# adhney/video-quierer

Hardware: AMD Instinct MI355X
Metric: frames/sec CLIP ViT-B/32 encode + queries/sec top-10 over 1M×512 embeds (higher is better)
Workload: dtype fp16 MFMA operands (every GEMM group), fp32 accumulate

## Files before the change

### video-quierer_amd/csrc/encoder_kernels.h

```cpp
#pragma once
#include "vq_common.h"
#include "gemm_mfma.h"

namespace vq {


template <bool F16>
__device__ __forceinline__ uint2 pack4_h(f32x4 v) {
    if constexpr (F16) {
        typedef __attribute__((ext_vector_type(4))) _Float16 h4;
        h4 b = {(_Float16)v[0], (_Float16)v[1], (_Float16)v[2], (_Float16)v[3]};
        return __builtin_bit_cast(uint2, b);
    } else {
        typedef __attribute__((ext_vector_type(4))) __bf16 bf16x4;
        bf16x4 b = {(__bf16)v[0], (__bf16)v[1], (__bf16)v[2], (__bf16)v[3]};
        return __builtin_bit_cast(uint2, b);
    }
}
template <bool F16>
__host__ __device__ inline uint16_t to_h16(float f) {
    if constexpr (F16) return __builtin_bit_cast(uint16_t, (_Float16)f);
    else return f32_to_bf16_rne(f);
}

// ... 342 lines not shown
#pragma unroll
    for (int i = 0; i < NV; ++i) {
        v[i].x -= mean; v[i].y -= mean; v[i].z -= mean; v[i].w -= mean;
        q += (v[i].x * v[i].x + v[i].y * v[i].y) + (v[i].z * v[i].z + v[i].w * v[i].w);
    }
    const float rstd = rsqrtf(wave_sum(q) / (float)hidden + eps);
#pragma unroll
    for (int i = 0; i < NV; ++i) {
        const float4 gg = *(const float4*)(g + (i * 64 + lane) * 4);
        const float4 bb = *(const float4*)(b + (i * 64 + lane) * 4);
        v[i].x = v[i].x * rstd * gg.x + bb.x; v[i].y = v[i].y * rstd * gg.y + bb.y;
        v[i].z = v[i].z * rstd * gg.z + bb.z; v[i].w = v[i].w * rstd * gg.w + bb.w;
    }
}

template <int NV, bool F16>
__global__ __launch_bounds__(256)
void layernorm_bf16_kernel(const float* __restrict__ x, uint16_t* __restrict__ h,
                           const float* __restrict__ g, const float* __restrict__ b,
                           int rows, float eps, int in_row_stride = 1) {
    constexpr int H = NV * 256;
    const int lane = threadIdx.x & 63;
    const int row = blockIdx.x * 4 + (threadIdx.x >> 6);
    if (row >= rows) return;
    float4 v[NV];
#pragma unroll
    for (int i = 0; i < NV; ++i) v[i] = *(const float4*)(x + (size_t)row * in_row_stride * H + (i * 64 + lane) * 4);
    ln_row<NV>(v, g, b, lane, eps, H);
#pragma unroll
    for (int i = 0; i < NV; ++i)
        *(uint2*)(h + (size_t)row * H + (i * 64 + lane) * 4) = pack4_h<F16>(f32x4{v[i].x, v[i].y, v[i].z, v[i].w});
}

template <int NV, bool F16>
__device__ __forceinline__ void emit_xh_and_partials(const float4 (&v)[NV], uint16_t* __restrict__ xh_row, LnPartials part,
                                                     int row, int lane) {
#pragma unroll
    for (int i = 0; i < NV; ++i) {
        *(uint2*)(xh_row + (i * 64 + lane) * 4) = pack4_h<F16>(f32x4{v[i].x, v[i].y, v[i].z, v[i].w});
        float s1 = (v[i].x + v[i].y) + (v[i].z + v[i].w);
        float s2 = (v[i].x * v[i].x + v[i].y * v[i].y) + (v[i].z * v[i].z + v[i].w * v[i].w);
        s1 = row16_sum(s1); s2 = row16_sum(s2);
        if ((lane & 15) == 0) part.ps[(size_t)(i * 4 + (lane >> 4)) * part.stride + row] = float2{s1, s2};
    }
}

template <int NV, bool F16>
__global__ __launch_bounds__(256)
void embed_finish_kernel(float* __restrict__ x, uint16_t* __restrict__ xh,
                         const float* __restrict__ cls, const float* __restrict__ pos0,
                         const float* __restrict__ g_pre, const float* __restrict__ b_pre,
                         LnPartials part, int rows, int tokens, float eps) {
    constexpr int H = NV * 256;
    const int lane = threadIdx.x & 63;
    const int row = blockIdx.x * 4 + (threadIdx.x >> 6);
    if (row >= rows) return;
    const bool is_cls = (row % tokens) == 0;
    float4 v[NV];
#pragma unroll
    for (int i = 0; i < NV; ++i) {
        const int o = (i * 64 + lane) * 4;
        if (is_cls) {
            const float4 c = *(const float4*)(cls + o), p = *(const float4*)(pos0 + o);
            v[i] = float4{c.x + p.x, c.y + p.y, c.z + p.z, c.w + p.w};
        } else {
            v[i] = *(const float4*)(x + (size_t)row * H + o);
        }
    }
    ln_row<NV>(v, g_pre, b_pre, lane, eps, H);
#pragma unroll
    for (int i = 0; i < NV; ++i) *(float4*)(x + (size_t)row * H + (i * 64 + lane) * 4) = v[i];
    emit_xh_and_partials<NV, F16>(v, xh + (size_t)row * H, part, row, lane);
}

inline __global__ __launch_bounds__(256)
void gather_rows_h16_kernel(const uint16_t* __restrict__ src, uint16_t* __restrict__ dst, int rows, int cols, int stride) {
    const int per_row = cols / 8;
    for (int i = blockIdx.x * blockDim.x + threadIdx.x; i < rows * per_row; i += gridDim.x * blockDim.x) {
        const int r = i / per_row, c = i - r * per_row;
        *(uint4*)(dst + (size_t)r * cols + c * 8) = *(const uint4*)(src + (size_t)r * stride * cols + c * 8);
    }
}

template <int NV, bool F16>
__global__ __launch_bounds__(256)
void embed_tokens_kernel(const int* __restrict__ ids, const float* __restrict__ tok, const float* __restrict__ pos,
                         float* __restrict__ x, uint16_t* __restrict__ xh, LnPartials part,
                         int rows, int seq, int vocab) {
    constexpr int H = NV * 256;
    const int lane = threadIdx.x & 63;
    const int row = blockIdx.x * 4 + (threadIdx.x >> 6);
    if (row >= rows) return;
    int id = ids[row];
    id = id < 0 ? 0 : (id >= vocab ? vocab - 1 : id);
    const int t = row % seq;
    float4 v[NV];
#pragma unroll
    for (int i = 0; i < NV; ++i) {
        const int o = (i * 64 + lane) * 4;
        const float4 a = *(const float4*)(tok + (size_t)id * H + o), p = *(const float4*)(pos + (size_t)t * H + o);
        v[i] = float4{a.x + p.x, a.y + p.y, a.z + p.z, a.w + p.w};
        *(float4*)(x + (size_t)row * H + o) = v[i];
    }
    emit_xh_and_partials<NV, F16>(v, xh + (size_t)row * H, part, row, lane);
}

inline __global__ void eos_rows_kernel(const int* __restrict__ ids, int* __restrict__ row_index, int n, int seq, int eos_id) {
    const int s = blockIdx.x * blockDim.x + threadIdx.x;
    if (s >= n) return;
    const int* p = ids + (size_t)s * seq;
    int pos = 0;
    if (eos_id == 2) {
        int best = p[0];
        for (int t = 1; t < seq; ++t) if (p[t] > best) { best = p[t]; pos = t; }
    } else {
        for (int t = 0; t < seq; ++t) if (p[t] == eos_id) { pos = t; break; }
    }
    row_index[s] = s * seq + pos;
}

#ifndef VQ_ATT_NT_LOAD
#define VQ_ATT_NT_LOAD 0
#endif
__device__ __forceinline__ uint4 ld16_att(const uint16_t* p) {
#if VQ_ATT_NT_LOAD
    typedef __attribute__((ext_vector_type(4))) unsigned int u32x4;
    const u32x4 v = __builtin_nontemporal_load((const u32x4*)p);
    return uint4{v[0], v[1], v[2], v[3]};
#else
    return *(const uint4*)p;
#endif
}

template <bool F16>
__global__ __launch_bounds__(256)
void attention_t64_kernel(const uint16_t* __restrict__ qkv, uint16_t* __restrict__ out,
                          int tokens, int hidden, int heads) {
    __shared__ __attribute__((aligned(16))) uint16_t vlds[4][64 * 64];
    const int lane = threadIdx.x & 63;
    const int wave = __builtin_amdgcn_readfirstlane(threadIdx.x >> 6);
    const int hgroups = heads >> 2;
    const int img = blockIdx.x / hgroups;
    const int head = (blockIdx.x - img * hgroups) * 4 + wave;
    const int ld = 3 * hidden;
    const uint16_t* base = qkv + (size_t)img * tokens * ld + head * 64;
    const int r16 = lane & 15, g = lane >> 4;
    typedef mfma_op<F16> op;
    typedef typename op::frag frag;

    uint16_t* vt = vlds[wave];
#pragma unroll
    for (int it = 0; it < 8; ++it) {
        const int id = it * 64 + lane, row = id >> 3, c = id & 7;
        uint4 val = {0u, 0u, 0u, 0u};
        if (row < tokens) val = ld16_att(base + 2 * hidden + (size_t)row * ld + c * 8);
        *(uint4*)(vt + row * 64 + c * 8) = val;
    }

    frag kf[4][2], qf[4][2];
#pragma unroll
    for (int t = 0; t < 4; ++t) {
        const int row = t * 16 + r16;
#pragma unroll
        for (int ks = 0; ks < 2; ++ks) {
            uint4 kv = {0u, 0u, 0u, 0u}, qv = {0u, 0u, 0u, 0u};
            if (row < tokens) {
// ... 18 lines not shown

    float inv_sum[4];
#pragma unroll
    for (int nt = 0; nt < 4; ++nt) {
        float mx = -3.0e38f;
#pragma unroll
        for (int mt = 0; mt < 4; ++mt)
#pragma unroll
            for (int r = 0; r < 4; ++r) {
                const int key = mt * 16 + g * 4 + r;
                if (key >= tokens) s[mt][nt][r] = -3.0e38f;
                mx = fmaxf(mx, s[mt][nt][r]);
            }
        mx = rows4_max(mx);
        float sum = 0.f;
#pragma unroll
        for (int mt = 0; mt < 4; ++mt)
#pragma unroll
            for (int r = 0; r < 4; ++r) {
                const float p = __expf(s[mt][nt][r] - mx);
                s[mt][nt][r] = p;
                sum += p;
            }
        sum = rows4_sum(sum);
        inv_sum[nt] = 1.0f / sum;
    }

    frag pf[4][2];
#pragma unroll
    for (int nt = 0; nt < 4; ++nt)
#pragma unroll
        for (int ss = 0; ss < 2; ++ss) {
            const f32x4 lo = s[2 * ss][nt], hi = s[2 * ss + 1][nt];
            const uint2 plo = pack4_h<F16>(lo), phi = pack4_h<F16>(hi);
            pf[nt][ss] = __builtin_bit_cast(frag, uint4{plo.x, plo.y, phi.x, phi.y});
        }

    __syncthreads();

    const int q4 = r16 >> 2, p4 = r16 & 3;
    typedef __attribute__((address_space(3))) s16x4 lds_s16x4;
#pragma unroll
    for (int dt = 0; dt < 4; ++dt) {
        f32x4 o[4];
#pragma unroll
        for (int nt = 0; nt < 4; ++nt) o[nt] = f32x4{0.f, 0.f, 0.f, 0.f};
#pragma unroll
        for (int ss = 0; ss < 2; ++ss) {
            const int key0 = 32 * ss + 4 * g + q4;
            const s16x4 lo = __builtin_amdgcn_ds_read_tr16_b64_v4i16(
                (lds_s16x4*)(vt + (key0) * 64 + dt * 16 + p4 * 4));
            const s16x4 hi = __builtin_amdgcn_ds_read_tr16_b64_v4i16(
                (lds_s16x4*)(vt + (key0 + 16) * 64 + dt * 16 + p4 * 4));
            typedef __attribute__((ext_vector_type(8))) short s16x8;
            const s16x8 both = {lo[0], lo[1], lo[2], lo[3], hi[0], hi[1], hi[2], hi[3]};
            const frag vf = __builtin_bit_cast(frag, both);
#pragma unroll
            for (int nt = 0; nt < 4; ++nt)
                o[nt] = op::run(vf, pf[nt][ss], o[nt]);
        }
#pragma unroll
        for (int nt = 0; nt < 4; ++nt) {
            const int qrow = nt * 16 + r16;
            if (qrow < tokens) {
                f32x4 v = o[nt];
                v[0] *= inv_sum[nt]; v[1] *= inv_sum[nt]; v[2] *= inv_sum[nt]; v[3] *= inv_sum[nt];
                *(uint2*)(out + ((size_t)img * tokens + qrow) * hidden + head * 64 + dt * 16 + g * 4) =
                    pack4_h<F16>(v);
            }
        }
    }
}

template <bool F16>
__device__ __forceinline__ typename mfma_op<F16>::frag ones_frag() {
    if constexpr (F16) { const _Float16 o = (_Float16)1.0f; return f16x8{o, o, o, o, o, o, o, o}; }
    else { const __bf16 o = (__bf16)1.0f; return bf16x8{o, o, o, o, o, o, o, o}; }
}
__device__ __forceinline__ uint4 buf_ld16(__amdgpu_buffer_rsrc_t r, int voff, int imm) {
    typedef __attribute__((ext_vector_type(4))) unsigned int u32x4;
    const u32x4 v = __builtin_amdgcn_raw_buffer_load_b128(r, voff + imm, 0, 0);
    return uint4{v[0], v[1], v[2], v[3]};
}
template <bool F16, int T>
__global__ __launch_bounds__(256, 2)
void attention_tile_kernel(const uint16_t* __restrict__ qkv, uint16_t* __restrict__ out, int hidden, int heads) {
    static_assert(T >= 17 && T <= 64, "single key tile of 64");
    __shared__ __attribute__((aligned(1024))) uint16_t vlds[4][64 * 64];
    typedef mfma_op<F16> op;
    typedef typename op::frag frag;
    typedef __attribute__((address_space(3))) void lds_void;
    const int lane = threadIdx.x & 63;
    const int wave = __builtin_amdgcn_readfirstlane(threadIdx.x >> 6);
    const int hgroups = heads >> 2;
    const int img = blockIdx.x / hgroups;
    const int head = (blockIdx.x - img * hgroups) * 4 + wave;
    const int ld = 3 * hidden;
    const int r16 = lane & 15, g = lane >> 4;
    const __amdgpu_buffer_rsrc_t src = __builtin_amdgcn_make_buffer_rsrc(
        (void*)(qkv + (size_t)img * T * ld + head * 64), 0, ((T - 1) * ld + 2 * hidden + 64) * 2, 0x00020000);
    const __amdgpu_buffer_rsrc_t dst = __builtin_amdgcn_make_buffer_rsrc(
        (void*)(out + (size_t)img * T * hidden + head * 64), 0, ((T - 1) * hidden + 64) * 2, 0x00020000);
    uint16_t* vt = vlds[wave];

    const int row_bytes = ld * 2;
    const int kq_off = r16 * row_bytes + g * 16;
    uint4 kraw[4][2], qraw[4][2];
#pragma unroll
    for (int t = 0; t < 4; ++t) {
        const int o = kq_off + t * 16 * row_bytes;
#pragma unroll
        for (int ks = 0; ks < 2; ++ks) {
            kraw[t][ks] = buf_ld16(src, o + hidden * 2, ks * 64);
            qraw[t][ks] = buf_ld16(src, o, ks * 64);
        }
    }
    constexpr int PIECES = (T + 7) / 8, ZROW0 = (T / 8) * 8;
    __builtin_amdgcn_sched_barrier(0);
    if constexpr (ZROW0 < 64) {
#pragma unroll
        for (int i = 0; i < (64 - ZROW0) * 128 / 1024; ++i)
            *(uint4*)(vt + ZROW0 * 64 + i * 512 + lane * 8) = uint4{0u, 0u, 0u, 0u};
    }
    const int v_off = (lane >> 3) * row_bytes + hidden * 4 + (((lane & 7) ^ (((lane >> 4) & 3) << 1)) << 4);
#pragma unroll
    for (int it = 0; it < PIECES; ++it) {
        if (it * 8 >= ZROW0) asm volatile("s_waitcnt lgkmcnt(0)" ::: "memory");
        __builtin_amdgcn_raw_ptr_buffer_load_lds(src, (lds_void*)(vt + it * 512), 16, v_off + it * 8 * row_bytes, 0, 0, 0);
    }
    __builtin_amdgcn_sched_barrier(0);

    frag kf[4][2], qf[4][2];
#pragma unroll
    for (int t = 0; t < 4; ++t)
#pragma unroll
        for (int ks = 0; ks < 2; ++ks) {
            kf[t][ks] = __builtin_bit_cast(frag, kraw[t][ks]);
            qf[t][ks] = __builtin_bit_cast(frag, qraw[t][ks]);
        }
    constexpr int KT = (T + 15) / 16;
    constexpr int FT = T / 16, R = T % 16;
    f32x4 s[4][4];
#pragma unroll
    for (int mt = 0; mt < KT; ++mt)
#pragma unroll
        for (int nt = 0; nt < 4; ++nt) {
            f32x4 a = {0.f, 0.f, 0.f, 0.f};
            a = op::run(kf[mt][0], qf[nt][0], a);
            a = op::run(kf[mt][1], qf[nt][1], a);
            s[mt][nt] = a;
        }
    const float NEGBIG = -3.0e38f, L2E = 1.44269504088896341f;
    float inv_sum[4];
#pragma unroll
    for (int nt = 0; nt < 4; ++nt) {
        float mx = NEGBIG;
#pragma unroll
        for (int mt = 0; mt < KT; ++mt)
#pragma unroll
            for (int r = 0; r < 4; ++r) {
                if (mt == FT) {
                    if (r >= R) continue;
                    if (4 * g + r >= R) s[mt][nt][r] = NEGBIG;
                }
                mx = fmaxf(mx, s[mt][nt][r]);
            }
        mx = rows4_max(mx);
        const float m2 = mx * L2E;
#pragma unroll
        for (int mt = 0; mt < KT; ++mt) {
            f32x4 e = s[mt][nt] * L2E - m2;
#pragma unroll
            for (int r = 0; r < 4; ++r) e[r] = (mt == FT && r >= R) ? 0.f : __builtin_amdgcn_exp2f(e[r]);
            s[mt][nt] = e;
        }
    }
    frag pf[4][2];
#pragma unroll
    for (int nt = 0; nt < 4; ++nt)
#pragma unroll
        for (int ss = 0; ss < 2; ++ss) {
            const uint2 plo = 2 * ss < KT ? pack4_h<F16>(s[2 * ss][nt]) : uint2{0u, 0u};
            const uint2 phi = 2 * ss + 1 < KT ? pack4_h<F16>(s[2 * ss + 1][nt]) : uint2{0u, 0u};
            pf[nt][ss] = __builtin_bit_cast(frag, uint4{plo.x, plo.y, phi.x, phi.y});
        }
    {
        const frag ones = ones_frag<F16>();
#pragma unroll
        for (int nt = 0; nt < 4; ++nt) {
            f32x4 d = {0.f, 0.f, 0.f, 0.f};
#pragma unroll
            for (int ss = 0; ss < 2; ++ss)
                if (2 * ss < KT) d = op::run(ones, pf[nt][ss], d);
            inv_sum[nt] = __builtin_amdgcn_rcpf(d[0]);
        }
    }

    __builtin_amdgcn_sched_barrier(0);
    asm volatile("s_waitcnt vmcnt(0)" ::: "memory");

    const int q4 = r16 >> 2, p4 = r16 & 3;
    const int sw = (2 * (g & 1) + (q4 >> 1)) & 3;
    typedef __attribute__((address_space(3))) s16x4 lds_s16x4;
    typedef __attribute__((ext_vector_type(8))) short s16x8;
    typedef __attribute__((ext_vector_type(4))) unsigned int u32x4;
    const int o_off = (r16 * hidden + g * 8) * 2;
#pragma unroll
    for (int a = 0; a < 2; ++a) {
        f32x4 o[2][4];
#pragma unroll
        for (int b = 0; b < 2; ++b) {
            const uint16_t* vrow = vt + (4 * g + q4) * 64 + (((4 * a + p4) ^ (sw << 1)) << 3) + 4 * b;
#pragma unroll
            for (int nt = 0; nt < 4; ++nt) o[b][nt] = f32x4{0.f, 0.f, 0.f, 0.f};
#pragma unroll
            for (int ss = 0; ss < 2; ++ss) {
                if (2 * ss >= KT) continue;
                const s16x4 lo = __builtin_amdgcn_ds_read_tr16_b64_v4i16((lds_s16x4*)(vrow + (32 * ss) * 64));
                s16x4 hi = {0, 0, 0, 0};
                if (2 * ss + 1 < KT) hi = __builtin_amdgcn_ds_read_tr16_b64_v4i16((lds_s16x4*)(vrow + (32 * ss + 16) * 64));
                const s16x8 both = {lo[0], lo[1], lo[2], lo[3], hi[0], hi[1], hi[2], hi[3]};
                const frag vf = __builtin_bit_cast(frag, both);
#pragma unroll
                for (int nt = 0; nt < 4; ++nt) o[b][nt] = op::run(vf, pf[nt][ss], o[b][nt]);
            }
        }
#pragma unroll
        for (int nt = 0; nt < 4; ++nt) {
            if (nt * 16 >= T) continue;
            const uint2 lo = pack4_h<F16>(o[0][nt] * inv_sum[nt]), hi = pack4_h<F16>(o[1][nt] * inv_sum[nt]);
            __builtin_amdgcn_raw_buffer_store_b128(u32x4{lo.x, lo.y, hi.x, hi.y}, dst, o_off + nt * 16 * hidden * 2 + a * 64, 0, 0);
        }
    }
}

template <bool F16, bool CAUSAL>
__global__ __launch_bounds__(256)
void attention_stream_kernel(const uint16_t* __restrict__ qkv, uint16_t* __restrict__ out,
                             int tokens, int hidden, int heads, int q_tiles, int total_units) {
    __shared__ __attribute__((aligned(16))) uint16_t vlds[4][64 * 64];
    typedef mfma_op<F16> op;
    typedef typename op::frag frag;
    const int lane = threadIdx.x & 63;
    const int wave = __builtin_amdgcn_readfirstlane(threadIdx.x >> 6);
    const int unit = blockIdx.x * 4 + wave;
    if (unit >= total_units) return;
    const int qt = unit % q_tiles;
    const int ih = unit / q_tiles;
    const int head = ih % heads, img = ih / heads;
    const int ld = 3 * hidden;
    const uint16_t* base = qkv + (size_t)img * tokens * ld + head * 64;
    const int r16 = lane & 15, g = lane >> 4;
    const int q0 = qt * 64;
    uint16_t* vt = vlds[wave];

    frag qf[4][2];
#pragma unroll
    for (int t = 0; t < 4; ++t) {
        const int row = q0 + t * 16 + r16;
#pragma unroll
        for (int ks = 0; ks < 2; ++ks) {
            uint4 qv = {0u, 0u, 0u, 0u};
            if (row < tokens) qv = *(const uint4*)(base + (size_t)row * ld + ks * 32 + g * 8);
            qf[t][ks] = __builtin_bit_cast(frag, qv);
        }
    }
    f32x4 o[4][4];
#pragma unroll
    for (int i = 0; i < 4; ++i)
#pragma unroll
        for (int j = 0; j < 4; ++j) o[i][j] = f32x4{0.f, 0.f, 0.f, 0.f};
    const float NEGBIG = -3.0e38f;
    float m_run[4] = {NEGBIG, NEGBIG, NEGBIG, NEGBIG}, l_run[4] = {0.f, 0.f, 0.f, 0.f};

    const int k_tiles = CAUSAL ? qt + 1 : (tokens + 63) / 64;
    const int q4 = r16 >> 2, p4 = r16 & 3;
    typedef __attribute__((address_space(3))) s16x4 lds_s16x4;
    typedef __attribute__((ext_vector_type(8))) short s16x8;

    for (int kt = 0; kt < k_tiles; ++kt) {
        const int k0 = kt * 64;
#pragma unroll
        for (int it = 0; it < 8; ++it) {
            const int id = it * 64 + lane, row = id >> 3, c = id & 7;
            uint4 val = {0u, 0u, 0u, 0u};
            if (k0 + row < tokens) val = *(const uint4*)(base + 2 * hidden + (size_t)(k0 + row) * ld + c * 8);
            *(uint4*)(vt + row * 64 + c * 8) = val;
        }
        frag kf[4][2];
#pragma unroll
        for (int t = 0; t < 4; ++t) {
            const int row = k0 + t * 16 + r16;
#pragma unroll
            for (int ks = 0; ks < 2; ++ks) {
                uint4 kv = {0u, 0u, 0u, 0u};
                if (row < tokens) kv = *(const uint4*)(base + hidden + (size_t)row * ld + ks * 32 + g * 8);
                kf[t][ks] = __builtin_bit_cast(frag, kv);
            }
        }
        f32x4 sc[4][4];
#pragma unroll
        for (int mt = 0; mt < 4; ++mt)
#pragma unroll
            for (int nt = 0; nt < 4; ++nt) {
                f32x4 a = {0.f, 0.f, 0.f, 0.f};
                a = op::run(kf[mt][0], qf[nt][0], a);
                a = op::run(kf[mt][1], qf[nt][1], a);
                sc[mt][nt] = a;
            }
        float alpha[4];
#pragma unroll
        for (int nt = 0; nt < 4; ++nt) {
            const int query = q0 + nt * 16 + r16;
            float mx = NEGBIG;
// ... 355 lines not shown
```

### video-quierer_amd/csrc/vq_encoder.hip

```cpp
#include "../../include/vq_amd.h"
#include "vq_common.h"
#include "gemm_dispatch.h"
#include "encoder_kernels.h"

#include <cmath>
#include <cstring>
#include <cstdlib>
#include <memory>
#include <mutex>
#include <type_traits>
#include <thread>
#include <algorithm>
#include <vector>

namespace vq {
int require_init();

enum EncClass { C_PATCHIFY = 0, C_GEMM_PATCH, C_EMBED_FINISH, C_LAYERNORM, C_GEMM_QKV, C_ATTENTION,
                C_GEMM_OUT, C_GEMM_FC1, C_GEMM_FC2, C_POOL, C_LAST_CLS };
static const char* kEncClassNames[VQ_ENC_NCLASS] = {
    "patchify_u8", "gemm_patch_embed", "embed_finish_ln", "layernorm_bf16", "gemm_qkv",
    "attention", "gemm_out_proj_residual", "gemm_fc1_quickgelu", "gemm_fc2_residual", "pool_project",
    "last_block_cls_rows"};

struct LayerW {
    float *c1_qkv, *c2_qkv, *b_out, *c1_fc1, *c2_fc1, *b_fc2;
    uint16_t *w_qkv, *w_out, *w_fc1, *w_fc2;
};

struct Arena {
    char* base = nullptr; size_t size = 0, used = 0;
    template <class T> T* take(size_t count) {
        used = (used + 255) & ~(size_t)255;
        T* p = (T*)(base + used);
        used += count * sizeof(T);
        return p;
    }
};

}

using namespace vq;

struct vq_encoder {
    vq_vit_config cfg{};
    int tokens = 0, patches = 0, grid = 0, patch_k = 0, max_batch = 0;
    int64_t rows_pad = 0, prow_pad = 0;
    hipStream_t stream = nullptr;
    hipStream_t own_stream = nullptr;
    std::mutex mu;
    Arena arena;
    std::shared_ptr<void> arena_owner;
    std::shared_ptr<void> weights_owner;
    uint16_t* w_patch = nullptr; float *b_patch = nullptr, *cls = nullptr, *pos = nullptr;
    float *pre_g = nullptr, *pre_b = nullptr, *post_g = nullptr, *post_b = nullptr, *w_proj = nullptr;
    std::vector<LayerW> layers;
    uint8_t* d_frames = nullptr;
    float *x = nullptr, *d_out = nullptr;
    uint16_t *h = nullptr, *qkv = nullptr, *att = nullptr, *mlp = nullptr;
    uint16_t* xl = nullptr;
    bool split_resid = true;
    float2* ps = nullptr;
    uint8_t* h_stage[2] = {nullptr, nullptr};
    float* h_out_stage = nullptr;
    uint8_t* d_slot_frames[2] = {nullptr, nullptr};
    float* h_slot_out[2] = {nullptr, nullptr};
    hipStream_t copy_stream = nullptr;
    hipEvent_t ev_h2d[2] = {nullptr, nullptr}, ev_fwd[2] = {nullptr, nullptr}, ev_done[2] = {nullptr, nullptr};
    int slot_n[2] = {0, 0};
    int run_layers = -1;
    bool keep_stream = false;
    bool stream_split = false;
    int last_n = 0;
    bool is_text = false;
    float* tok_emb = nullptr; int* d_ids = nullptr; int* d_rowidx = nullptr; int vocab = 0, eos_id = 0;
    bool attn_simple = false;
    bool attn_q64 = false;
    bool attn_t64 = false;
    bool prune_last = true;
    float patch_unscale = 1.0f;
    int f16_mask = 0;
    bool h_is_f16 = false;
    int gemm24_mask = 0;
    int gemm_force = GK_AUTO;
    bool profiling = false;
    struct Ev { int cls; hipEvent_t a, b; };
    std::vector<Ev> events;
    std::vector<hipEvent_t> pool;
};

namespace {

struct Prof {
    vq_encoder* e; int cls; hipEvent_t a = nullptr, b = nullptr;
    static hipEvent_t get(vq_encoder* e) {
        if (!e->pool.empty()) { hipEvent_t ev = e->pool.back(); e->pool.pop_back(); return ev; }
        hipEvent_t ev; (void)hipEventCreate(&ev); return ev;
    }
    Prof(vq_encoder* enc, int c) : e(enc), cls(c) {
        if (e->profiling) { a = get(e); b = get(e); (void)hipEventRecord(a, e->stream); }
    }
    ~Prof() {
        if (e->profiling) { (void)hipEventRecord(b, e->stream); e->events.push_back({cls, a, b}); }
    }
};

size_t arena_bytes(const vq_vit_config& c, int tokens, int patches, int patch_k, int max_batch,
                   int64_t rows_pad, int64_t prow_pad) {
    size_t h = c.hidden, m = c.mlp, n = 0;
    auto add = [&](size_t bytes) { n = ((n + 255) & ~(size_t)255) + bytes; };
    add((size_t)h * patch_k * 2); add(h * 4); add(h * 4); add((size_t)tokens * h * 4);
    add(h * 4); add(h * 4); add(h * 4); add(h * 4); add((size_t)c.proj_dim * h * 4);
    for (int l = 0; l < c.layers; ++l) {
        add(3 * h * 4); add(3 * h * 4); add(h * 4); add(m * 4); add(m * 4); add(h * 4);
        add(3 * h * h * 2); add(h * h * 2); add(m * h * 2); add(h * m * 2);
    }
    add((size_t)max_batch * c.image_size * c.image_size * 3);
    add((size_t)LN_MAX_GRANULES * rows_pad * 8);
    add((size_t)rows_pad * h * 4); add((size_t)max_batch * c.proj_dim * 4);
    add((size_t)rows_pad * h * 2); add((size_t)rows_pad * h * 2); add((size_t)rows_pad * 3 * h * 2); add((size_t)rows_pad * h * 2);
    size_t mlp_elems = std::max((size_t)rows_pad * m, (size_t)prow_pad * patch_k);
    add(mlp_elems * 2);
    (void)patches;
    return n + 4096;
}

int upload_f32(float* dst, const float* src, size_t n) {
    VQ_HIP(hipMemcpy(dst, src, n * 4, hipMemcpyHostToDevice));
    return 0;
}
int upload_h16(uint16_t* dst, const float* src, size_t n, bool f16, float scale = 1.0f) {
    std::vector<uint16_t> tmp(n);
    if (f16) for (size_t i = 0; i < n; ++i) tmp[i] = __builtin_bit_cast(uint16_t, (_Float16)(src[i] * scale));
    else     for (size_t i = 0; i < n; ++i) tmp[i] = f32_to_bf16_rne(src[i] * scale);
    VQ_HIP(hipMemcpy(dst, tmp.data(), n * 2, hipMemcpyHostToDevice));
    return 0;
}

enum : int { DT_PATCH = 1, DT_QKV = 2, DT_ATTN = 4, DT_FC1 = 8, DT_FC2 = 16, DT_ALL = 31 };

int upload_folded(uint16_t* dst, float* c1_dst, float* c2_dst, const float* W, const float* gamma, const float* beta,
                  const float* bias, size_t N, size_t K, bool f16, float scale = 1.0f) {
    std::vector<uint16_t> w16(N * K);
    std::vector<float> c1(N), c2(N);
    for (size_t n = 0; n < N; ++n) {
        double s1 = 0.0, s2 = 0.0;
        for (size_t k = 0; k < K; ++k) {
            const float wf = W[n * K + k] * scale * gamma[k];
            const uint16_t r = f16 ? __builtin_bit_cast(uint16_t, (_Float16)wf) : f32_to_bf16_rne(wf);
            w16[n * K + k] = r;
            s1 += f16 ? (double)(float)__builtin_bit_cast(_Float16, r) : (double)bf16_to_f32(r);
            s2 += (double)beta[k] * (double)W[n * K + k];
        }
        c1[n] = (float)s1;
        c2[n] = (float)((s2 + (double)bias[n]) * (double)scale);
    }
    VQ_HIP(hipMemcpy(dst, w16.data(), w16.size() * 2, hipMemcpyHostToDevice));
    VQ_HIP(hipMemcpy(c1_dst, c1.data(), N * 4, hipMemcpyHostToDevice));
    VQ_HIP(hipMemcpy(c2_dst, c2.data(), N * 4, hipMemcpyHostToDevice));
    return 0;
}

// ... 35 lines not shown
    hipStream_t st = e->stream;
    const int H = c.hidden, T = e->tokens;
    const int rows = n * T;
    const bool fP = e->f16_mask & DT_PATCH, fQ = e->f16_mask & DT_QKV, fA = e->f16_mask & DT_ATTN,
               f1 = e->f16_mask & DT_FC1, f2 = e->f16_mask & DT_FC2;
    auto pad_rows = [](int r) {
        const int r256 = (int)round_up(r, G2_BM), r128 = (int)round_up(r, GEMM_BM);
        return (r256 - r128) * 16 <= r128 ? r256 : r128;
    };
    const int rows_gemm = pad_rows(rows);
    auto use24 = [&](int bit, int M, int N, int K) {
        return (e->gemm24_mask & bit) && (e->gemm_force == GK_AUTO || e->gemm_force == GK_AUTO_NO160) && M % G2_BM == 0 && N % G2_BN == 0 && K % (2 * G2_BK) == 0 &&
               (int64_t)(M / G2_BM) * (N / G2_BN) >= 128;
    };
    auto gemm_rows = [&](int N, int K, int bit = 0) {
        if (use24(bit, rows_gemm, N, K)) return rows_gemm;
        const int r160 = (int)round_up(rows, G5_BM);
        return (e->gemm_force == GK_AUTO && gemm_use160() && r160 <= e->rows_pad && prefer_tn160(r160, N, K)) ? r160 : rows_gemm;
    };
    auto gf = [&](int bit, int M, int N, int K) { return use24(bit, M, N, K) ? (int)GK_ASM256 : e->gemm_force; };
    const int prows = n * e->patches;
    const int prows_gemm = pad_rows(prows);
    const LnPartials part{e->ps, e->rows_pad};
    const int granules = H / 64;
    const float inv_h = 1.0f / (float)H;

    const int nl = e->run_layers < 0 ? c.layers : std::min(e->run_layers, c.layers);
    if (e->is_text) {
        Prof p(e, C_EMBED_FINISH);
        by_f16(fQ, [&](auto F) {
            hipLaunchKernelGGL((embed_tokens_kernel<NV, VQ_F16(F)>), dim3(cdiv(rows, 4)), dim3(256), 0, st, d_ids, e->tok_emb,
                               e->pos, e->x, e->h, part, rows, T, e->vocab);
            return 0;
        });
        hipLaunchKernelGGL(eos_rows_kernel, dim3(cdiv(n, 256)), dim3(256), 0, st, d_ids, e->d_rowidx, n, T, e->eos_id);
    } else {
    {
        Prof p(e, C_PATCHIFY);
        by_f16(fP, [&](auto F) {
            if (c.patch_size % 8 == 0 && e->patch_k == 3 * c.patch_size * c.patch_size) {
                const int64_t total = (int64_t)n * c.image_size * (c.image_size / 8);
                const int blocks = (int)std::min<int64_t>((total + 255) / 256, 256 * 16);
                hipLaunchKernelGGL(patchify_u8_kernel<VQ_F16(F)>, dim3(blocks), dim3(256), 0, st, d_frames, e->mlp, n,
                                   c.image_size, c.patch_size, swap_rb);
            } else {
                const int64_t total = (int64_t)n * e->patches * 3 * c.patch_size;
                const int blocks = (int)std::min<int64_t>((total + 255) / 256, 256 * 16);
                hipLaunchKernelGGL(patchify_generic_kernel<VQ_F16(F)>, dim3(blocks), dim3(256), 0, st, d_frames, e->mlp, n,
                                   c.image_size, c.patch_size, e->patch_k, swap_rb);
            }
            return 0;
        });
    }
    {
        Prof p(e, C_GEMM_PATCH);
        VQ_TRY(by_f16(fP, [&](auto F) {
            return launch_gemm_auto<VQ_F16(F)>(st, e->mlp, e->patch_k, e->w_patch, e->patch_k, prows_gemm, H, e->patch_k,
                                               EpiPatchEmbedF32{e->x, H, e->b_patch, e->pos, e->patches, T, prows, e->patch_unscale}, gf(16, prows_gemm, H, e->patch_k));
        }));
    }
    {
        Prof p(e, C_EMBED_FINISH);
        by_f16(fQ, [&](auto F) {
            hipLaunchKernelGGL((embed_finish_kernel<NV, VQ_F16(F)>), dim3(cdiv(rows, 4)), dim3(256), 0, st, e->x, e->h, e->cls,
                               e->pos, e->pre_g, e->pre_b, part, rows, T, c.ln_eps);
            return 0;
        });
    }
    }
    e->h_is_f16 = fQ;
    const bool as_full = e->run_layers < 0 || e->keep_stream;
    const int last_l = as_full ? c.layers - 1 : nl - 1;
    const bool cls_last = !e->is_text && e->prune_last && as_full;
    const bool split = e->split_resid && fQ && f1 && as_full;
    bool stream_split = false;
    auto resid_mode = [&](bool wants_f32_after) {
        if (!split) return (int)RS_F32;
        const int m = (stream_split ? RS_IN_SPLIT : 0) | (wants_f32_after ? RS_OUT_F32 : RS_OUT_SPLIT);
        stream_split = !wants_f32_after;
        return m;
    };
    for (int l = 0; l < nl; ++l) {
        const LayerW& L = e->layers[l];
        {
            Prof p(e, C_GEMM_QKV);
            VQ_TRY(by_f16(fQ, [&](auto F) {
                return by_f16(fA, [&](auto FO) {
                    return launch_gemm_auto<VQ_F16(F)>(st, e->h, H, L.w_qkv, H, rows_gemm, 3 * H, H,
                                                       EpiLnH16<VQ_F16(FO), false>{e->qkv, 3 * H, L.c2_qkv, L.c1_qkv, part, granules, inv_h, c.ln_eps},
                                                       gf(1, rows_gemm, 3 * H, H));
                });
            }));
        }
        {
            Prof p(e, C_ATTENTION);
            by_f16(fA, [&](auto F) {
                constexpr bool F16 = VQ_F16(F);
                if (e->is_text) {
                    const int q_tiles = cdiv(T, 64), q_groups = cdiv(q_tiles, 4);
                    hipLaunchKernelGGL((attention_stream_wg_kernel<F16, true>), dim3(n * c.heads * q_groups), dim3(256), 0, st,
                                       e->qkv, e->att, T, H, c.heads, q_tiles, q_groups);
                } else if (T == 50 && c.heads % 4 == 0 && !e->attn_t64) {
                    hipLaunchKernelGGL((attention_tile_kernel<F16, 50>), dim3(n * (c.heads / 4)), dim3(256), 0, st, e->qkv, e->att, H, c.heads);
                } else if (T <= 64 && c.heads % 4 == 0) {
                    hipLaunchKernelGGL(attention_t64_kernel<F16>, dim3(n * (c.heads / 4)), dim3(256), 0, st, e->qkv, e->att, T, H,
                                       c.heads);
                } else {
                    const int q_tiles = cdiv(T, 64), q_groups = cdiv(q_tiles, 4);
                    if (e->attn_simple) {
                        const int units = n * c.heads * q_tiles;
                        hipLaunchKernelGGL((attention_stream_kernel<F16, false>), dim3(cdiv(units, 4)), dim3(256), 0, st, e->qkv,
                                           e->att, T, H, c.heads, q_tiles, units);
                    } else if (!e->attn_q64) {
                        const int q_tiles32 = cdiv(T, 32), q_groups32 = cdiv(q_tiles32, 4);
                        hipLaunchKernelGGL((attention_stream_wg_kernel<F16, false, 2>), dim3(n * c.heads * q_groups32), dim3(256), 0, st,
                                           e->qkv, e->att, T, H, c.heads, q_tiles32, q_groups32);
                    } else {
                        hipLaunchKernelGGL((attention_stream_wg_kernel<F16, false>), dim3(n * c.heads * q_groups), dim3(256), 0, st,
                                           e->qkv, e->att, T, H, c.heads, q_tiles, q_groups);
                    }
                }
                return 0;
            });
        }
        const bool cls_only = cls_last && l == c.layers - 1;
        if (cls_only) {
            const int crows = pad_rows(n);
            {
                Prof p(e, C_LAST_CLS);
                hipLaunchKernelGGL(gather_rows_h16_kernel, dim3(cdiv(n * (H / 8), 256)), dim3(256), 0, st, e->att, e->qkv, n, H, T);
                VQ_TRY(by_f16(fA, [&](auto F) {
                    return by_f16(f1, [&](auto FO) {
                        return launch_gemm_auto<VQ_F16(F)>(st, e->qkv, H, L.w_out, H, crows, H, H,
                                                           EpiBiasResidualClsLnF32<VQ_F16(FO)>{e->x, H, T, L.b_out, n, e->h, part}, e->gemm_force);
                    });
                }));
                e->h_is_f16 = f1;
            }
            {
                Prof p(e, C_LAST_CLS);
                VQ_TRY(by_f16(f1, [&](auto F) {
                    return by_f16(f2, [&](auto FO) {
                        return launch_gemm_auto<VQ_F16(F)>(st, e->h, H, L.w_fc1, H, crows, c.mlp, H,
                                                           EpiLnH16<VQ_F16(FO), true>{e->mlp, c.mlp, L.c2_fc1, L.c1_fc1, part, granules, inv_h, c.ln_eps},
                                                           e->gemm_force);
                    });
                }));
            }
            {
                Prof p(e, C_LAST_CLS);
                const int splits = (c.mlp % (8 * GEMM_BK) == 0 && (size_t)8 * crows * H * 2 <= (size_t)e->rows_pad * 3 * H) ? 8 : 0;
                if (splits && crows % GEMM_BM == 0 && e->gemm_force != GK_PHASE4 && e->gemm_force != GK_DEEP) {
                    float* part = (float*)e->qkv;
                    const int64_t plane = (int64_t)crows * H;
                    VQ_TRY(by_f16(f2, [&](auto F) {
                        return launch_gemm_tn_splitk<VQ_F16(F)>(st, e->mlp, c.mlp, L.w_fc2, c.mlp, crows, H, c.mlp, splits,
                                                                EpiSplitKPartialF32{part, H, plane});
                    }));
                    hipLaunchKernelGGL(splitk_reduce_residual_cls_kernel, dim3(cdiv((int64_t)n * (H / 4), 256)), dim3(256), 0, st, part, plane,
                                       splits, e->x, L.b_fc2, H, T, n);
                } else {
                    VQ_TRY(by_f16(f2, [&](auto F) {
                        return launch_gemm_auto<VQ_F16(F)>(st, e->mlp, c.mlp, L.w_fc2, c.mlp, crows, H, c.mlp,
                                                           EpiBiasResidualClsF32{e->x, H, T, L.b_fc2, n}, e->gemm_force);
                    }));
                }
            }
            continue;
        }
        {
            Prof p(e, C_GEMM_OUT);
            const int mode = resid_mode(false);
            VQ_TRY(by_f16(fA, [&](auto F) {
                return by_f16(f1, [&](auto FO) {
                    auto go = [&](auto epi) { return launch_gemm_auto<VQ_F16(F)>(st, e->att, H, L.w_out, H, gemm_rows(H, H, 2), H, H, epi, gf(2, rows_gemm, H, H)); };
                    if constexpr (VQ_F16(FO)) {
                        if (mode == RS_OUT_SPLIT) return go(EpiBiasResidualLnF32<0, true, RS_OUT_SPLIT>{e->x, H, L.b_out, e->h, part, e->xl});
                        if (mode == (RS_IN_SPLIT | RS_OUT_SPLIT)) return go(EpiBiasResidualLnF32<0, true, RS_IN_SPLIT | RS_OUT_SPLIT>{e->x, H, L.b_out, e->h, part, e->xl});
                    }
                    return go(EpiBiasResidualLnF32<0, VQ_F16(FO)>{e->x, H, L.b_out, e->h, part});
                });
            }));
            e->h_is_f16 = f1;
        }
        {
            Prof p(e, C_GEMM_FC1);
            VQ_TRY(by_f16(f1, [&](auto F) {
                return by_f16(f2, [&](auto FO) {
                    return launch_gemm_auto<VQ_F16(F)>(st, e->h, H, L.w_fc1, H, rows_gemm, c.mlp, H,
                                                       EpiLnH16<VQ_F16(FO), true>{e->mlp, c.mlp, L.c2_fc1, L.c1_fc1, part, granules, inv_h, c.ln_eps},
                                                       gf(4, rows_gemm, c.mlp, H));
                });
            }));
        }
        {
            Prof p(e, C_GEMM_FC2);
            const int mode = resid_mode(l == last_l || (cls_last && l == c.layers - 2));
            VQ_TRY(by_f16(f2, [&](auto F) {
                return by_f16(fQ, [&](auto FO) {
                    auto go = [&](auto epi) { return launch_gemm_auto<VQ_F16(F)>(st, e->mlp, c.mlp, L.w_fc2, c.mlp, gemm_rows(H, c.mlp, 8), H, c.mlp, epi, gf(8, rows_gemm, H, c.mlp)); };
                    if constexpr (VQ_F16(FO)) {
                        if (mode == (RS_IN_SPLIT | RS_OUT_SPLIT)) return go(EpiBiasResidualLnF32<1, true, RS_IN_SPLIT | RS_OUT_SPLIT>{e->x, H, L.b_fc2, e->h, part, e->xl});
                        if (mode == (RS_IN_SPLIT | RS_OUT_F32)) return go(EpiBiasResidualLnF32<1, true, RS_IN_SPLIT | RS_OUT_F32>{e->x, H, L.b_fc2, e->h, part, e->xl});
                    }
                    return go(EpiBiasResidualLnF32<1, VQ_F16(FO)>{e->x, H, L.b_fc2, e->h, part});
                });
            }));
            e->h_is_f16 = fQ;
        }
    }
    {
        Prof p(e, C_POOL);
        hipLaunchKernelGGL((pool_project_kernel<NV>), dim3(cdiv(n, POOL_IMGS), cdiv(c.proj_dim, POOL_CHUNK)), dim3(256), 0, st,
                           e->x, e->post_g, e->post_b, e->w_proj, d_out_f32, n, T, c.proj_dim, c.ln_eps,
                           e->is_text ? e->d_rowidx : (const int*)nullptr);
        hipLaunchKernelGGL(l2_normalize_rows_kernel, dim3(cdiv(n, 4)), dim3(256), 0, st, d_out_f32, d_out_f16, n, c.proj_dim);
    }
    VQ_HIP(hipGetLastError());
    e->last_n = n;
    e->stream_split = stream_split;
    return 0;
}

int forward(vq_encoder* e, const uint8_t* d_frames, int n, int swap_rb, float* d_out_f32, uint16_t* d_out_f16,
            const int* d_ids = nullptr) {
    switch (e->cfg.hidden / 256) {
        case 2: return run_forward<2>(e, d_frames, n, swap_rb, d_out_f32, d_out_f16, d_ids);
        case 3: return run_forward<3>(e, d_frames, n, swap_rb, d_out_f32, d_out_f16, d_ids);
        case 4: return run_forward<4>(e, d_frames, n, swap_rb, d_out_f32, d_out_f16, d_ids);
        default: return fail(VQ_ERR_INVALID, "unsupported hidden size %d", e->cfg.hidden);
    }
}

int dtype_mask_from(int flags) {
    int mask = (flags & VQ_ENC_FP16) ? DT_ALL : ((flags >> 8) & DT_ALL);
    if (const char* dt = getenv("VQ_AMD_DTYPE")) {
        if (!strcmp(dt, "fp16") || !strcmp(dt, "f16")) mask = DT_ALL;
        else if (!strcmp(dt, "bf16")) mask = 0;
        else if (!strcmp(dt, "mixed")) mask = (VQ_ENC_MIXED >> 8) & DT_ALL;
        else if (!strncmp(dt, "mask:", 5)) mask = atoi(dt + 5) & DT_ALL;
    }
    return mask;
}

void apply_create_options(vq_encoder* e, int flags, const vq_encoder* parent) {
    if (!e->is_text && (flags & VQ_ENC_CONCURRENT)) e->gemm_force = GK_AUTO_NO160;
    if (const char* gf = getenv("VQ_AMD_GEMM")) e->gemm_force = atoi(gf);
    if (const char* rs = getenv("VQ_AMD_RESID")) e->split_resid = strcmp(rs, "f32") != 0;
#ifdef VQ_DIAG
    if (const char* gm = getenv("VQ_AMD_GEMM24")) e->gemm24_mask = atoi(gm);
#endif
    if (parent) {
        e->attn_simple = parent->attn_simple; e->attn_q64 = parent->attn_q64; e->attn_t64 = parent->attn_t64; e->prune_last = parent->prune_last;
        e->f16_mask = parent->f16_mask;
        return;
    }
    if (!e->is_text) {
        if (const char* at = getenv("VQ_AMD_ATTN")) { e->attn_simple = !strcmp(at, "simple"); e->attn_q64 = !strcmp(at, "q64"); e->attn_t64 = !strcmp(at, "t64"); }
        if (const char* fl = getenv("VQ_AMD_FULL_LAST_LAYER")) e->prune_last = atoi(fl) == 0;
    }
    e->f16_mask = dtype_mask_from(flags);
}

}

extern "C" {

int vq_encoder_create(const vq_vit_config* cfg, const float* const* weights, int n_weights, int max_batch,
                      vq_encoder** out) {
    return vq_encoder_create_ex(cfg, weights, n_weights, max_batch, 0, out);
}

int vq_encoder_create_ex(const vq_vit_config* cfg, const float* const* weights, int n_weights, int max_batch,
                         int flags, vq_encoder** out) {
    VQ_TRY(require_init());
    VQ_CHECK(cfg && weights && out, "vq_encoder_create: null argument");
    const vq_vit_config c = *cfg;
    VQ_CHECK(c.layers > 0 && n_weights == 5 + 16 * c.layers + 3, "vq_encoder_create: expected %d weight tensors, got %d",
             5 + 16 * c.layers + 3, n_weights);
    VQ_CHECK(max_batch > 0 && max_batch <= 8192, "vq_encoder_create: max_batch %d out of range", max_batch);
    VQ_CHECK(c.image_size > 0 && c.patch_size > 0 && c.image_size % c.patch_size == 0,
             "vq_encoder_create: image %d is not a multiple of patch %d", c.image_size, c.patch_size);
    const int grid = c.image_size / c.patch_size, patches = grid * grid, tokens = patches + 1;
    VQ_CHECK(tokens <= 4096, "vq_encoder_create: %d tokens is beyond what this build sizes for", tokens);
    VQ_CHECK(c.hidden % c.heads == 0 && c.hidden / c.heads == 64, "vq_encoder_create: head_dim must be 64");
    VQ_CHECK((c.hidden == 768 || c.hidden == 1024) && c.mlp % 128 == 0, "vq_encoder_create: hidden %d / mlp %d unsupported",
             c.hidden, c.mlp);
    VQ_CHECK(c.proj_dim > 0 && c.proj_dim <= 4096, "vq_encoder_create: proj_dim %d out of range", c.proj_dim);
    const int patch_k_raw = 3 * c.patch_size * c.patch_size;
    const int patch_k = (int)round_up(patch_k_raw, 2 * G2_BK);

    vq_encoder* e = new vq_encoder();
    apply_create_options(e, flags, nullptr);
    e->cfg = c; e->tokens = tokens; e->patches = patches; e->grid = grid; e->patch_k = patch_k; e->max_batch = max_batch;
    e->rows_pad = round_up((int64_t)max_batch * tokens + (G5_BM - 1), 256);
    e->prow_pad = round_up((int64_t)max_batch * patches, 256);
    auto cleanup = [&](int rc) { vq_encoder_destroy(e); return rc; };

    const size_t bytes = arena_bytes(c, tokens, patches, patch_k, max_batch, e->rows_pad, e->prow_pad);
    hipError_t he = hipMalloc((void**)&e->arena.base, bytes);
    if (he != hipSuccess) { delete e; return fail(VQ_ERR_OOM, "vq_encoder_create: hipMalloc(%zu) failed: %s", bytes, hipGetErrorString(he)); }
    e->arena.size = bytes;
    e->arena_owner = std::shared_ptr<void>(e->arena.base, [](void* p) { (void)hipFree(p); });
    he = hipMemset(e->arena.base, 0, bytes);
    if (he != hipSuccess) return cleanup(fail(VQ_ERR_HIP, "hipMemset failed: %s", hipGetErrorString(he)));
    he = hipStreamCreateWithFlags(&e->own_stream, hipStreamNonBlocking);
    if (he != hipSuccess) return cleanup(fail(VQ_ERR_HIP, "hipStreamCreate failed: %s", hipGetErrorString(he)));
    e->stream = e->own_stream;

    Arena& A = e->arena;
    const size_t H = c.hidden, M = c.mlp;
    int wi = 0;
    int rc = 0;
#define UP(expr) do { rc = (expr); if (rc) return cleanup(rc); } while (0)
    static const double mean[3] = {0.48145466, 0.4578275, 0.40821073};
    static const double stdv[3] = {0.26862954, 0.26130258, 0.27577711};
    e->cls = A.take<float>(H);                UP(upload_f32(e->cls, weights[wi++], H));
    {
        const float* wp = weights[wi++];
        const int pp = c.patch_size * c.patch_size;
        std::vector<uint16_t> w16(H * patch_k);
        std::vector<float> bias(H);
        int pshift = 0;
        if (e->f16_mask & DT_PATCH) {
            double amax = 0.0;
            for (size_t n = 0; n < H; ++n)
                for (int ch = 0; ch < 3; ++ch)
                    for (int i = 0; i < pp; ++i) amax = std::max(amax, std::fabs((double)wp[(n * 3 + ch) * pp + i]) / (255.0 * stdv[ch]));
            if (amax > 0.0 && std::isfinite(amax)) pshift = std::min(24, std::max(0, (int)std::floor(std::log2(16000.0 / amax))));
        }
        e->patch_unscale = (float)std::ldexp(1.0, -pshift);
        const double pscale = std::ldexp(1.0, pshift);
        for (size_t n = 0; n < H; ++n) {
            double b = 0.0;
            for (int ch = 0; ch < 3; ++ch)
                for (int i = 0; i < pp; ++i) {
                    const double w = wp[(n * 3 + ch) * pp + i];
                    w16[n * patch_k + ch * pp + i] = (e->f16_mask & DT_PATCH) ? __builtin_bit_cast(uint16_t, (_Float16)(float)(w * pscale / (255.0 * stdv[ch])))
                                                             : f32_to_bf16_rne((float)(w / (255.0 * stdv[ch])));
                    b += w * (128.0 / 255.0 - mean[ch]) / stdv[ch];
                }
            bias[n] = (float)b;
// ... 474 lines not shown
```

Baseline: 108,400.

## Compute only CLS queries in last ViT layer attention

In the final layer, where only the CLS token output is needed, the QKV GEMM now computes K and V for all tokens but Q only for the gathered CLS rows. A CLS-specialised attention tile kernel then processes a single query tile and writes the CLS output straight into a compact buffer, which removes the later gather. The intent is to cut about a third of the last-layer QKV GEMM work and most of its attention compute. The cost is an extra gather kernel for the CLS rows and LN partials, plus reuse of the MLP scratch buffer.

Result: no change. 109,200 (median of 6 runs) (+0.8%).

```diff
diff --git a/video-quierer_amd/csrc/encoder_kernels.h b/video-quierer_amd/csrc/encoder_kernels.h
--- a/video-quierer_amd/csrc/encoder_kernels.h
+++ b/video-quierer_amd/csrc/encoder_kernels.h
@@ -448,6 +448,27 @@
     }
 }
 
+inline __global__ __launch_bounds__(256)
+void gather_cls_rows_kernel(const uint16_t* __restrict__ xh, LnPartials part, uint16_t* __restrict__ xhc, float2* __restrict__ psc,
+                            uint16_t* __restrict__ zc, int rows, int rows_pad, int cols, int tokens) {
+    const int per_row = cols / 8;
+    const int n_x = rows_pad * per_row, n_p = LN_MAX_GRANULES * rows_pad;
+    for (int i = blockIdx.x * blockDim.x + threadIdx.x; i < n_x + n_p; i += gridDim.x * blockDim.x) {
+        if (i < n_x) {
+            const int r = i / per_row, c = i - r * per_row;
+            if (r < rows) {
+                *(uint4*)(xhc + (size_t)r * cols + c * 8) = *(const uint4*)(xh + (size_t)r * tokens * cols + c * 8);
+            } else {
+                *(uint4*)(xhc + (size_t)r * cols + c * 8) = uint4{0u, 0u, 0u, 0u};
+                *(uint4*)(zc + (size_t)r * cols + c * 8) = uint4{0u, 0u, 0u, 0u};
+            }
+        } else {
+            const int j = i - n_x, g = j / rows_pad, r = j - g * rows_pad;
+            psc[j] = r < rows ? part.ps[(size_t)g * part.stride + (size_t)r * tokens] : float2{0.f, 0.f};
+        }
+    }
+}
+
 template <int NV, bool F16>
 __global__ __launch_bounds__(256)
 void embed_tokens_kernel(const int* __restrict__ ids, const float* __restrict__ tok, const float* __restrict__ pos,
@@ -632,9 +653,11 @@
     const u32x4 v = __builtin_amdgcn_raw_buffer_load_b128(r, voff + imm, 0, 0);
     return uint4{v[0], v[1], v[2], v[3]};
 }
-template <bool F16, int T>
+template <bool F16, int T, bool CLS = false>
 __global__ __launch_bounds__(256, 2)
-void attention_tile_kernel(const uint16_t* __restrict__ qkv, uint16_t* __restrict__ out, int hidden, int heads) {
+void attention_tile_kernel(const uint16_t* __restrict__ qkv, uint16_t* __restrict__ out, int hidden, int heads,
+                           const uint16_t* __restrict__ qc = nullptr, uint16_t* __restrict__ outc = nullptr) {
+    constexpr int NT = CLS ? 1 : 4;
     static_assert(T >= 17 && T <= 64, "single key tile of 64");
     __shared__ __attribute__((aligned(1024))) uint16_t vlds[4][64 * 64];
     typedef mfma_op<F16> op;
@@ -650,7 +673,9 @@
     const __amdgpu_buffer_rsrc_t src = __builtin_amdgcn_make_buffer_rsrc(
         (void*)(qkv + (size_t)img * T * ld + head * 64), 0, ((T - 1) * ld + 2 * hidden + 64) * 2, 0x00020000);
     const __amdgpu_buffer_rsrc_t dst = __builtin_amdgcn_make_buffer_rsrc(
-        (void*)(out + (size_t)img * T * hidden + head * 64), 0, ((T - 1) * hidden + 64) * 2, 0x00020000);
+        (void*)(out + (size_t)img * T * hidden + head * 64), 0, CLS ? 64 * 2 : ((T - 1) * hidden + 64) * 2, 0x00020000);
+    const __amdgpu_buffer_rsrc_t qsrc = CLS ? __builtin_amdgcn_make_buffer_rsrc((void*)(qc + (size_t)img * hidden + head * 64), 0, 64 * 2, 0x00020000) : src;
+    const __amdgpu_buffer_rsrc_t dstc = CLS ? __builtin_amdgcn_make_buffer_rsrc((void*)(outc + (size_t)img * hidden + head * 64), 0, 64 * 2, 0x00020000) : dst;
     uint16_t* vt = vlds[wave];
 
     const int row_bytes = ld * 2;
@@ -662,7 +687,7 @@
 #pragma unroll
         for (int ks = 0; ks < 2; ++ks) {
             kraw[t][ks] = buf_ld16(src, o + hidden * 2, ks * 64);
-            qraw[t][ks] = buf_ld16(src, o, ks * 64);
+            if (t < NT) qraw[t][ks] = buf_ld16(qsrc, o, ks * 64);
         }
     }
     constexpr int PIECES = (T + 7) / 8, ZROW0 = (T / 8) * 8;
@@ -686,7 +711,7 @@
 #pragma unroll
         for (int ks = 0; ks < 2; ++ks) {
             kf[t][ks] = __builtin_bit_cast(frag, kraw[t][ks]);
-            qf[t][ks] = __builtin_bit_cast(frag, qraw[t][ks]);
+            if (t < NT) qf[t][ks] = __builtin_bit_cast(frag, qraw[t][ks]);
         }
     constexpr int KT = (T + 15) / 16;
     constexpr int FT = T / 16, R = T % 16;
@@ -694,7 +719,7 @@
 #pragma unroll
     for (int mt = 0; mt < KT; ++mt)
 #pragma unroll
-        for (int nt = 0; nt < 4; ++nt) {
+        for (int nt = 0; nt < NT; ++nt) {
             f32x4 a = {0.f, 0.f, 0.f, 0.f};
             a = op::run(kf[mt][0], qf[nt][0], a);
             a = op::run(kf[mt][1], qf[nt][1], a);
@@ -703,7 +728,7 @@
     const float NEGBIG = -3.0e38f, L2E = 1.44269504088896341f;
     float inv_sum[4];
 #pragma unroll
-    for (int nt = 0; nt < 4; ++nt) {
+    for (int nt = 0; nt < NT; ++nt) {
         float mx = NEGBIG;
 #pragma unroll
         for (int mt = 0; mt < KT; ++mt)
@@ -727,7 +752,7 @@
     }
     frag pf[4][2];
 #pragma unroll
-    for (int nt = 0; nt < 4; ++nt)
+    for (int nt = 0; nt < NT; ++nt)
 #pragma unroll
         for (int ss = 0; ss < 2; ++ss) {
             const uint2 plo = 2 * ss < KT ? pack4_h<F16>(s[2 * ss][nt]) : uint2{0u, 0u};
@@ -737,7 +762,7 @@
     {
         const frag ones = ones_frag<F16>();
 #pragma unroll
-        for (int nt = 0; nt < 4; ++nt) {
+        for (int nt = 0; nt < NT; ++nt) {
             f32x4 d = {0.f, 0.f, 0.f, 0.f};
 #pragma unroll
             for (int ss = 0; ss < 2; ++ss)
@@ -762,7 +787,7 @@
         for (int b = 0; b < 2; ++b) {
             const uint16_t* vrow = vt + (4 * g + q4) * 64 + (((4 * a + p4) ^ (sw << 1)) << 3) + 4 * b;
 #pragma unroll
-            for (int nt = 0; nt < 4; ++nt) o[b][nt] = f32x4{0.f, 0.f, 0.f, 0.f};
+            for (int nt = 0; nt < NT; ++nt) o[b][nt] = f32x4{0.f, 0.f, 0.f, 0.f};
 #pragma unroll
             for (int ss = 0; ss < 2; ++ss) {
                 if (2 * ss >= KT) continue;
@@ -772,14 +797,15 @@
                 const s16x8 both = {lo[0], lo[1], lo[2], lo[3], hi[0], hi[1], hi[2], hi[3]};
                 const frag vf = __builtin_bit_cast(frag, both);
 #pragma unroll
-                for (int nt = 0; nt < 4; ++nt) o[b][nt] = op::run(vf, pf[nt][ss], o[b][nt]);
-            }
-        }
-#pragma unroll
-        for (int nt = 0; nt < 4; ++nt) {
+                for (int nt = 0; nt < NT; ++nt) o[b][nt] = op::run(vf, pf[nt][ss], o[b][nt]);
+            }
+        }
+#pragma unroll
+        for (int nt = 0; nt < NT; ++nt) {
             if (nt * 16 >= T) continue;
             const uint2 lo = pack4_h<F16>(o[0][nt] * inv_sum[nt]), hi = pack4_h<F16>(o[1][nt] * inv_sum[nt]);
             __builtin_amdgcn_raw_buffer_store_b128(u32x4{lo.x, lo.y, hi.x, hi.y}, dst, o_off + nt * 16 * hidden * 2 + a * 64, 0, 0);
+            if constexpr (CLS) __builtin_amdgcn_raw_buffer_store_b128(u32x4{lo.x, lo.y, hi.x, hi.y}, dstc, o_off + a * 64, 0, 0);
         }
     }
 }
diff --git a/video-quierer_amd/csrc/vq_encoder.hip b/video-quierer_amd/csrc/vq_encoder.hip
--- a/video-quierer_amd/csrc/vq_encoder.hip
+++ b/video-quierer_amd/csrc/vq_encoder.hip
@@ -78,6 +78,7 @@
     bool attn_q64 = false;
     bool attn_t64 = false;
     bool prune_last = true;
+    bool trim_last_qkv = true;
     float patch_unscale = 1.0f;
     int f16_mask = 0;
     bool h_is_f16 = false;
@@ -279,6 +280,48 @@
     };
     for (int l = 0; l < nl; ++l) {
         const LayerW& L = e->layers[l];
+        const bool cls_only = cls_last && l == c.layers - 1;
+        const int crows = pad_rows(n);
+        const size_t cplane = (size_t)crows * H;
+        const bool trim = cls_only && e->trim_last_qkv && T == 50 && c.heads % 4 == 0 && !e->attn_t64 &&
+                          3 * cplane * 2 + (size_t)LN_MAX_GRANULES * crows * sizeof(float2) <= (size_t)e->rows_pad * c.mlp * 2;
+        uint16_t *q_c = e->mlp, *xh_c = e->mlp + cplane, *att_c = e->mlp + 2 * cplane;
+        if (trim) {
+            float2* ps_c = (float2*)(e->mlp + 3 * cplane);
+            {
+                Prof p(e, C_LAST_CLS);
+                hipLaunchKernelGGL(gather_cls_rows_kernel, dim3(cdiv(crows * (H / 8 + LN_MAX_GRANULES), 256)), dim3(256), 0, st, e->h, part, xh_c,
+                                   ps_c, att_c, n, crows, H, T);
+            }
+            {
+                Prof p(e, C_LAST_CLS);
+                VQ_TRY(by_f16(fQ, [&](auto F) {
+                    return by_f16(fA, [&](auto FO) {
+                        return launch_gemm_auto<VQ_F16(F)>(st, e->h, H, L.w_qkv + (size_t)H * H, H, rows_gemm, 2 * H, H,
+                                                           EpiLnH16<VQ_F16(FO), false>{e->qkv + H, 3 * H, L.c2_qkv + H, L.c1_qkv + H, part, granules, inv_h, c.ln_eps},
+                                                           gf(1, rows_gemm, 2 * H, H));
+                    });
+                }));
+            }
+            {
+                Prof p(e, C_LAST_CLS);
+                VQ_TRY(by_f16(fQ, [&](auto F) {
+                    return by_f16(fA, [&](auto FO) {
+                        return launch_gemm_auto<VQ_F16(F)>(st, xh_c, H, L.w_qkv, H, crows, H, H,
+                                                           EpiLnH16<VQ_F16(FO), false>{q_c, H, L.c2_qkv, L.c1_qkv, LnPartials{ps_c, crows}, granules, inv_h, c.ln_eps},
+                                                           e->gemm_force);
+                    });
+                }));
+            }
+            {
+                Prof p(e, C_LAST_CLS);
+                by_f16(fA, [&](auto F) {
+                    hipLaunchKernelGGL((attention_tile_kernel<VQ_F16(F), 50, true>), dim3(n * (c.heads / 4)), dim3(256), 0, st, e->qkv, e->att, H, c.heads,
+                                       q_c, att_c);
+                    return 0;
+                });
+            }
+        } else {
         {
             Prof p(e, C_GEMM_QKV);
             VQ_TRY(by_f16(fQ, [&](auto F) {
@@ -320,15 +363,15 @@
                 return 0;
             });
         }
-        const bool cls_only = cls_last && l == c.layers - 1;
+        }
         if (cls_only) {
-            const int crows = pad_rows(n);
             {
                 Prof p(e, C_LAST_CLS);
-                hipLaunchKernelGGL(gather_rows_h16_kernel, dim3(cdiv(n * (H / 8), 256)), dim3(256), 0, st, e->att, e->qkv, n, H, T);
+                const uint16_t* att_cls = trim ? att_c : e->qkv;
+                if (!trim) hipLaunchKernelGGL(gather_rows_h16_kernel, dim3(cdiv(n * (H / 8), 256)), dim3(256), 0, st, e->att, e->qkv, n, H, T);
                 VQ_TRY(by_f16(fA, [&](auto F) {
                     return by_f16(f1, [&](auto FO) {
-                        return launch_gemm_auto<VQ_F16(F)>(st, e->qkv, H, L.w_out, H, crows, H, H,
+                        return launch_gemm_auto<VQ_F16(F)>(st, att_cls, H, L.w_out, H, crows, H, H,
                                                            EpiBiasResidualClsLnF32<VQ_F16(FO)>{e->x, H, T, L.b_out, n, e->h, part}, e->gemm_force);
                     });
                 }));
@@ -448,13 +491,14 @@
     if (const char* gm = getenv("VQ_AMD_GEMM24")) e->gemm24_mask = atoi(gm);
 #endif
     if (parent) {
-        e->attn_simple = parent->attn_simple; e->attn_q64 = parent->attn_q64; e->attn_t64 = parent->attn_t64; e->prune_last = parent->prune_last;
+        e->attn_simple = parent->attn_simple; e->attn_q64 = parent->attn_q64; e->attn_t64 = parent->attn_t64; e->prune_last = parent->prune_last; e->trim_last_qkv = parent->trim_last_qkv;
         e->f16_mask = parent->f16_mask;
         return;
     }
     if (!e->is_text) {
         if (const char* at = getenv("VQ_AMD_ATTN")) { e->attn_simple = !strcmp(at, "simple"); e->attn_q64 = !strcmp(at, "q64"); e->attn_t64 = !strcmp(at, "t64"); }
         if (const char* fl = getenv("VQ_AMD_FULL_LAST_LAYER")) e->prune_last = atoi(fl) == 0;
+        if (const char* lq = getenv("VQ_AMD_LAST_QKV")) e->trim_last_qkv = strcmp(lq, "full") != 0;
     }
     e->f16_mask = dtype_mask_from(flags);
 }
```
